# zillow/salve

Measured on AMD Instinct MI355X. Metric: alignment hypotheses/sec (render+verify), higher is better.
Workload: dtype fp16

## Files before the change

### include/salve_hip.h

```cpp
#ifndef SALVE_HIP_H
#define SALVE_HIP_H

#include <stddef.h>
#include <stdint.h>

#ifdef __cplusplus
extern "C" {
#endif

typedef enum {
    SALVE_OK = 0,
    SALVE_ERR_BAD_ARG = -1,
    SALVE_ERR_UNSUPPORTED = -2,
    SALVE_ERR_HIP = -3,
    SALVE_ERR_WORKSPACE = -4
} salve_status_t;

#define SALVE_HIP_ABI_VERSION 7

#define SALVE_STATUS_WALK_FAILED 1
#define SALVE_STATUS_FP16_RANGE 2
#define SALVE_STATUS_BAD_HYPOTHESIS 4

#define SALVE_STATUS_LAYOUT_THICKNESS 8
// ... 78 lines not shown
    int32_t reserved;
    float R[4], t[2];
    double s;
} salve_layout_pose_t;
int salve_layout_pose(const double* room_xy, const int64_t* room_off, int64_t n_room_xy, const double* wdo_xy, const uint8_t* wdo_type,
                      const int64_t* wdo_off, int64_t n_wdo, int32_t n_panos, const salve_layout_pose_t* recs, int32_t n,
                      double bev_tx, double bev_ty, double bev_scale, int32_t line_width, salve_layout_t* layouts, int32_t* poly_xy,
                      int32_t poly_cap, int32_t* segs, int32_t seg_cap, int32_t* status, void* stream);

int salve_bev_export_u8(const uint32_t* bev, int32_t n, int32_t bev_h, int32_t bev_w, uint8_t* out, void* stream);

typedef struct {
    int64_t bev_offset;
    int32_t slot;
    int32_t chan;
} salve_tile_job_t;

#define SALVE_TILE_F32_NCHW 0
#define SALVE_TILE_F16_NHWC 1
#define SALVE_TILE_U8X4 2

int salve_bev_tiles(const uint32_t* bev, int32_t bev_h, int32_t bev_w, const salve_tile_job_t* jobs, int32_t n_jobs,
                    const int32_t* coef_y, const int32_t* coef_x, int32_t resize, int32_t crop, const float* lut,
                    void* out, int32_t out_format, int32_t out_c, void* stream);

typedef struct {
    int32_t crop_y, crop_x;
    int32_t flags;
    int32_t reserved;
} salve_tile_aug_t;
#define SALVE_TILE_HFLIP 1
#define SALVE_TILE_VFLIP 2
int salve_bev_tiles_aug(const uint32_t* bev, int32_t bev_h, int32_t bev_w, const salve_tile_job_t* jobs, const salve_tile_aug_t* aug,
                        int32_t n_jobs, const int32_t* coef_y, const int32_t* coef_x, int32_t resize, int32_t crop, const float* lut,
                        float* out, int32_t out_c, void* stream);

#define SALVE_TILE_F32_NHWC 3
#define SALVE_TILE_BF16_NHWC 4
int salve_bev_train_tiles(const uint32_t* bev_a, int32_t n_bev_a, const uint32_t* bev_b, int32_t n_bev_b, int32_t bev_h, int32_t bev_w,
                          const salve_tile_job_t* jobs_a, const salve_tile_job_t* jobs_b, int32_t per_sample, const salve_tile_aug_t* aug,
                          int32_t batch, const int32_t* coef_y, const int32_t* coef_x, int32_t resize, int32_t crop, const float* lut,
                          void* out, int32_t out_format, int32_t out_c, int32_t* status, void* stream);

int salve_bev_tile_pairs(const uint32_t* bev_a, const uint32_t* bev_b, int32_t bev_h, int32_t bev_w, const salve_tile_job_t* jobs_a,
                         const salve_tile_job_t* jobs_b, int32_t n_pairs, const int32_t* coef_y, const int32_t* coef_x, int32_t resize,
                         int32_t crop, const float* lut, void* out, int32_t out_c, int32_t b_pretiled, void* stream);

int salve_bev_densify_tiles(const salve_bev_config_t* cfg, int32_t n, uint32_t* out_bev, const salve_tile_job_t* jobs_a, const salve_tile_job_t* jobs_b,
                            const uint32_t* tiles_b, const int32_t* coef_y, const int32_t* coef_x, int32_t resize, int32_t crop, const float* lut,
                            void* out, int32_t out_c, int32_t* status, void* workspace, size_t workspace_bytes, void* stream);

#define SALVE_OP_CONV 0
#define SALVE_OP_MAXPOOL 1
#define SALVE_OP_AVGPOOL_FC 2
#define SALVE_NET_INPUT (-1)
#define SALVE_NO_BUF (-2)

typedef struct {
    int32_t op;
    int32_t in_buf, out_buf, res_buf;
    int32_t Hi, Wi, Cin;
    int32_t Ho, Wo, Cout;
    int32_t KH, KW, stride, pad;
    int32_t relu, reserved;
    int64_t w_off;
    int64_t b_off;
    int64_t ktab_off;
    int32_t in2_buf, Cin2, stride2, Hi2, Wi2, reserved2;
} salve_resnet_op_t;

#define SALVE_RESNET_CONV_IGEMM_ONLY 1
#define SALVE_RESNET_CONV8_WHEREVER 2
#define SALVE_RESNET_ROUND_ROBIN_TILES 4
#define SALVE_RESNET_NO_STEM_FUSE 8
#define SALVE_RESNET_NO_BLOCK_FUSE 16
#define SALVE_RESNET_NO_PROJ_FUSE 32
#define SALVE_RESNET_NO_CHAIN 64
#define SALVE_RESNET_CHAIN_EXPAND_ONLY 128
#define SALVE_RESNET_CHAIN_16_WAVES 256
#define SALVE_RESNET_CHAIN_NO_SPLIT 512
#define SALVE_RESNET_CHAIN_STORE_ALL 1024
#define SALVE_RESNET_NO_TRANSPOSED_TILES 2048
#define SALVE_RESNET_NO_NEXT_FUSE 4096
#define SALVE_RESNET_ALL_FLAGS 8191

void* salve_resnet_create(int32_t num_layers, int32_t in_channels, const salve_resnet_op_t* ops, int32_t n_ops,
                          const void* weights_f16, size_t weights_bytes, const float* params_f32, size_t params_bytes,
                          const int32_t* ktab, size_t ktab_entries, int32_t flags);
void salve_resnet_destroy(void* handle);
int salve_resnet_num_layers(void* handle);
size_t salve_resnet_workspace_bytes(void* handle, int32_t batch);
int salve_resnet_forward(void* handle, const void* input, int32_t batch, float* logits, void* workspace,
                         size_t workspace_bytes, int32_t* status, void* stream);

void* salve_resnet_f32_create(int32_t num_layers, int32_t in_channels, const salve_resnet_op_t* ops, int32_t n_ops,
                              const float* weights_f32, size_t weights_bytes, const float* params_f32, size_t params_bytes,
                              const int32_t* ktab, size_t ktab_entries, int32_t flags);
void salve_resnet_f32_destroy(void* handle);
size_t salve_resnet_f32_workspace_bytes(void* handle, int32_t batch);
int salve_resnet_f32_forward(void* handle, const float* input, int32_t batch, float* logits, void* workspace,
                             size_t workspace_bytes, int32_t* status, void* stream);

typedef struct {
    int32_t batch, Hi, Wi, Cin, Ho, Wo, Cout, KH, KW, stride, pad;
} salve_conv_desc_t;
#define SALVE_CONV_FWD 0
#define SALVE_CONV_DGRAD 1
#define SALVE_CONV_WGRAD 2
size_t salve_conv_f32_workspace_bytes(const salve_conv_desc_t* d, int32_t pass);
int salve_conv_f32_forward(const salve_conv_desc_t* d, const float* x, const float* w, float* y, void* ws, size_t ws_bytes, void* stream);
int salve_conv_f32_backward_data(const salve_conv_desc_t* d, const float* dy, const float* w, float* dx, void* ws, size_t ws_bytes,
                                 void* stream);
int salve_conv_f32_backward_weight(const salve_conv_desc_t* d, const float* x, const float* dy, float* dw, void* ws, size_t ws_bytes,
                                   void* stream);

size_t salve_conv_bf16_workspace_bytes(const salve_conv_desc_t* d, int32_t pass);
int salve_conv_bf16_forward(const salve_conv_desc_t* d, const uint16_t* x, const uint16_t* w, uint16_t* y, void* ws, size_t ws_bytes,
                            void* stream);
int salve_conv_bf16_backward_data(const salve_conv_desc_t* d, const uint16_t* dy, const uint16_t* w, uint16_t* dx, void* ws, size_t ws_bytes,
                                  void* stream);
int salve_conv_bf16_backward_weight(const salve_conv_desc_t* d, const uint16_t* x, const uint16_t* dy, float* dw, void* ws, size_t ws_bytes,
                                    void* stream);

typedef struct {
    int32_t rows, C, flags;
    float eps, momentum;
} salve_bn_desc_t;
#define SALVE_BN_RELU 1
#define SALVE_BN_ADD 2
#define SALVE_BN_EVAL 4
#define SALVE_BN_FWD 0
#define SALVE_BN_BWD 1
size_t salve_bn_workspace_bytes(const salve_bn_desc_t* d, int32_t pass);
int salve_bn_f32_forward(const salve_bn_desc_t* d, const float* x, const float* residual, const float* gamma, const float* beta,
                         float* running_mean, float* running_var, float* y, float* save_mean, float* save_invstd, void* ws, size_t ws_bytes,
                         void* stream);
int salve_bn_f32_backward(const salve_bn_desc_t* d, const float* dy, const float* x, const float* y, const float* gamma, const float* save_mean,
                          const float* save_invstd, float* dx, float* dres, float* dgamma, float* dbeta, void* ws, size_t ws_bytes, void* stream);
int salve_bn_bf16_forward(const salve_bn_desc_t* d, const uint16_t* x, const uint16_t* residual, const float* gamma, const float* beta,
                          float* running_mean, float* running_var, uint16_t* y, float* save_mean, float* save_invstd, void* ws, size_t ws_bytes,
                          void* stream);
int salve_bn_bf16_backward(const salve_bn_desc_t* d, const uint16_t* dy, const uint16_t* x, const uint16_t* y, const float* gamma,
                           const float* save_mean, const float* save_invstd, uint16_t* dx, uint16_t* dres, float* dgamma, float* dbeta, void* ws,
                           size_t ws_bytes, void* stream);

#define SALVE_ADAM_CHUNK 4096
typedef struct {
    float* param;
    const float* grad;
    float* exp_avg;
    float* exp_avg_sq;
    uint16_t* shadow_bf16;
    int64_t n;
    float step_size, sqrt_bc2, beta1, beta2, eps, weight_decay, one_minus_beta1, one_minus_beta2;
} salve_adam_segment_t;
typedef struct {
    int32_t segment, reserved;
    int64_t offset;
} salve_adam_chunk_t;
int salve_adam_step(const salve_adam_segment_t* table, int32_t n_segments, const salve_adam_chunk_t* chunk_map, int32_t n_chunks,
                    const salve_adam_segment_t* host_table, const salve_adam_chunk_t* host_chunk_map, void* stream);

#define SALVE_HEAD_MAX_CLASSES 16
typedef struct {
    int32_t B, HW, C, K, flags;
} salve_head_desc_t;
typedef struct {
// ... 24 lines not shown
```

### salve_amd/_lib.py

```python

from __future__ import annotations

import ctypes
from pathlib import Path

import numpy as np

import os

LIB_PATH = Path(os.environ.get("SALVE_HIP_LIB") or (Path(__file__).resolve().parent / "libsalve_hip.so"))

SALVE_OK = 0
EXPECTED_ABI = 7
TILE_F32_NCHW = 0
TILE_F16_NHWC = 1
TILE_U8X4 = 2
TILE_F32_NHWC = 3
TILE_BF16_NHWC = 4

EXPORTED_SYMBOLS = (
    "salve_hip_version",
    "salve_last_error",
    "salve_bev_workspace_bytes",
    "salve_bev_pano_index_bytes",
    "salve_bev_pano_index_build",
    "salve_bev_render_batch",
    "salve_bev_scatter",
    "salve_bev_densify",
    "salve_bev_scatter_points",
    "salve_zorder_winners",
    "salve_remove_hallucinated",
    "salve_bev_keys_from_pixels",
    "salve_bev_export_u8",
    "salve_layout_rasterise",
    "salve_bev_tiles",
    "salve_bev_tile_pairs",
    "salve_bev_densify_tiles",
    "salve_resize_rgb_u8",
    "salve_resnet_create",
    "salve_resnet_destroy",
    "salve_resnet_workspace_bytes",
    "salve_resnet_forward",
    "salve_resnet_num_layers",
    "salve_resnet_f32_create",
    "salve_resnet_f32_destroy",
    "salve_resnet_f32_workspace_bytes",
    "salve_resnet_f32_forward",
    "salve_bev_tiles_aug",
    "salve_conv_f32_workspace_bytes",
    "salve_conv_f32_forward",
    "salve_conv_f32_backward_data",
    "salve_conv_f32_backward_weight",
    "salve_conv_bf16_workspace_bytes",
    "salve_conv_bf16_forward",
    "salve_conv_bf16_backward_data",
    "salve_conv_bf16_backward_weight",
    "salve_bn_workspace_bytes",
    "salve_bn_f32_forward",
    "salve_bn_f32_backward",
    "salve_bn_bf16_forward",
    "salve_bn_bf16_backward",
    "salve_bev_train_tiles",
    "salve_bev_pano_index_update",
    "salve_layout_pose",
    "salve_adam_step",
    "salve_head_workspace_bytes",
    "salve_head_f32_forward",
    "salve_head_f32_backward",
    "salve_head_bf16_forward",
    "salve_head_bf16_backward",
)
RESNET_CONV_IGEMM_ONLY, RESNET_CONV8_WHEREVER, RESNET_ROUND_ROBIN_TILES, RESNET_NO_STEM_FUSE, RESNET_NO_BLOCK_FUSE = 1, 2, 4, 8, 16
RESNET_NO_PROJ_FUSE, RESNET_NO_CHAIN, RESNET_CHAIN_EXPAND_ONLY, RESNET_CHAIN_16_WAVES, RESNET_CHAIN_NO_SPLIT = 32, 64, 128, 256, 512
RESNET_CHAIN_STORE_ALL, RESNET_NO_TRANSPOSED_TILES, RESNET_NO_NEXT_FUSE = 1024, 2048, 4096
STATUS_WALK_FAILED = 1
STATUS_FP16_RANGE = 2
STATUS_BAD_HYPOTHESIS = 4
STATUS_LAYOUT_THICKNESS = 8
STATUS_BAD_TILE_JOB = 16
STATUS_BAD_PANO_SLOT = 32
STATUS_BAD_LAYOUT = 64


class BevConfig(ctypes.Structure):

    _fields_ = [
        ("pano_h", ctypes.c_int32), ("pano_w", ctypes.c_int32), ("crop_rows", ctypes.c_int32),
        ("bev_h", ctypes.c_int32), ("bev_w", ctypes.c_int32), ("mask_k", ctypes.c_int32),
        ("depth_scale", ctypes.c_float), ("out_flags", ctypes.c_int32),
        ("win_xmin", ctypes.c_double), ("win_xmax", ctypes.c_double),
        ("win_ymin", ctypes.c_double), ("win_ymax", ctypes.c_double),
        ("img_tx", ctypes.c_double), ("img_ty", ctypes.c_double), ("img_scale", ctypes.c_double),
        ("rot_pre", ctypes.c_double * 4),
        ("z_lo", ctypes.c_double * 2), ("z_hi", ctypes.c_double * 2),
        ("z_min", ctypes.c_double), ("n_slices", ctypes.c_int32), ("reserved1", ctypes.c_int32),
    ]


HYP_DTYPE = np.dtype(
    [("pano_idx", "<i4"), ("surface", "<i4"), ("R", "<f4", (4,)), ("t", "<f4", (2,)), ("apply_pose", "<i4"),
     ("reserved", "<i4")]
)
TILE_JOB_DTYPE = np.dtype([("bev_offset", "<i8"), ("slot", "<i4"), ("chan", "<i4")])
LAYOUT_DTYPE = np.dtype([("n_poly", "<i4"), ("poly_off", "<i4"), ("n_seg", "<i4"), ("seg_off", "<i4")])
LAYOUT_POSE_DTYPE = np.dtype([("pano", "<i4"), ("poly_off", "<i4"), ("seg_off", "<i4"), ("reserved", "<i4"), ("R", "<f4", (4,)), ("t", "<f4", (2,)),
                              ("s", "<f8")])
TILE_AUG_DTYPE = np.dtype([("crop_y", "<i4"), ("crop_x", "<i4"), ("flags", "<i4"), ("reserved", "<i4")])
TILE_HFLIP, TILE_VFLIP = 1, 2
assert LAYOUT_POSE_DTYPE.itemsize == 48 and HYP_DTYPE.itemsize == 40 and TILE_JOB_DTYPE.itemsize == 16 and TILE_AUG_DTYPE.itemsize == 16

CONV_FWD, CONV_DGRAD, CONV_WGRAD = 0, 1, 2
SALVE_ERR_BAD_ARG, SALVE_ERR_UNSUPPORTED = -1, -2


class ConvDesc(ctypes.Structure):

    _fields_ = [(n, ctypes.c_int32) for n in ("batch", "Hi", "Wi", "Cin", "Ho", "Wo", "Cout", "KH", "KW", "stride", "pad")]


BN_RELU, BN_ADD, BN_EVAL = 1, 2, 4
BN_FWD, BN_BWD = 0, 1


class BnDesc(ctypes.Structure):

    _fields_ = [("rows", ctypes.c_int32), ("C", ctypes.c_int32), ("flags", ctypes.c_int32), ("eps", ctypes.c_float),
                ("momentum", ctypes.c_float)]


ADAM_CHUNK = 4096
ADAM_SEGMENT_DTYPE = np.dtype([("param", "<u8"), ("grad", "<u8"), ("exp_avg", "<u8"), ("exp_avg_sq", "<u8"), ("shadow_bf16", "<u8"), ("n", "<i8"),
                               ("step_size", "<f4"), ("sqrt_bc2", "<f4"), ("beta1", "<f4"), ("beta2", "<f4"), ("eps", "<f4"),
                               ("weight_decay", "<f4"), ("one_minus_beta1", "<f4"), ("one_minus_beta2", "<f4")])
ADAM_CHUNK_DTYPE = np.dtype([("segment", "<i4"), ("reserved", "<i4"), ("offset", "<i8")])
assert ADAM_SEGMENT_DTYPE.itemsize == 80 and ADAM_CHUNK_DTYPE.itemsize == 16

HEAD_MAX_CLASSES = 16
HEAD_ACCUMULATE_LOSS = 1
HEAD_FWD, HEAD_BWD = 0, 1
HEAD_METER_DTYPE = np.dtype([("total", "<i8", (HEAD_MAX_CLASSES,)), ("correct", "<i8", (HEAD_MAX_CLASSES,)), ("loss_sum", "<f8"), ("loss_rows", "<i8"),
                             ("bad_targets", "<i8")])
assert HEAD_METER_DTYPE.itemsize == 280


class HeadDesc(ctypes.Structure):

    _fields_ = [(n, ctypes.c_int32) for n in ("B", "HW", "C", "K", "flags")]


_lib = None


class SalveHipError(RuntimeError):
    pass


def load() -> ctypes.CDLL:
# ... 132 lines not shown
```

### salve_amd/csrc/conv8.h

```cpp

constexpr int C8_THREADS = 512;
constexpr int C8_BM = 256, C8_BN = 256, C8_KS = 64;
constexpr int C8_HALF_E = 128 * C8_KS;

#define C8_MFMA(B_, A_, C_) { C_ = __builtin_amdgcn_mfma_f32_16x16x32_f16(B_, A_, C_, 0, 0, 0); }

template <bool POINTWISE, bool SRC2>
__global__ __launch_bounds__(C8_THREADS, 2) void conv8_kernel(ConvArgs p) {
    constexpr int BM = C8_BM, BN = C8_BN, KS = C8_KS;
    constexpr int LDC = BN + 8;
    constexpr int RING_E = 8 * C8_HALF_E, C_E = BM * LDC;
    __shared__ __attribute__((aligned(1024))) uint16_t smem[RING_E > C_E ? RING_E : C_E];

    int m_tile, n_tile;
    if (!xcd_tile(blockIdx.x, p.m_tiles, p.n_tiles, p.xcd_contig, m_tile, n_tile)) return;
    const int tid = threadIdx.x, lane = tid & 63, wave = __builtin_amdgcn_readfirstlane(tid >> 6);
    const int wr = wave >> 2, wc = wave & 3;
    const int m0 = m_tile * BM, n0 = n_tile * BN;
    const int r8 = tid >> 3;
    const int chunk = (tid & 7) ^ ((r8 >> 1) & 7);

    int iy0[2][2], ix0[2][2];
    const uint16_t* rowp[2][2];
    const uint16_t* rowp2[2][2];
// ... 123 lines not shown
    asm volatile("s_waitcnt vmcnt(8)" ::: "memory");
    __builtin_amdgcn_s_barrier();
    if (wave >= 4) __builtin_amdgcn_s_barrier();
    for (int kt = 0; kt < nkt; kt++) {
        C8_PHASE_HEAD({ C8_READ_A(kt, 0); C8_READ_B(bf0, kt, 1); }, C8_STAGE(kt + 1, 2));
        C8_WAIT_BARRIER();
        C8_MULT(0, bf0, 0);
        __builtin_amdgcn_s_barrier();
        C8_PHASE_HEAD({ C8_READ_B(bf1, kt, 2); }, C8_STAGE(kt + 1, 3));
        C8_WAIT_BARRIER();
        C8_MULT(0, bf1, 1);
        __builtin_amdgcn_s_barrier();
        C8_PHASE_HEAD({ C8_READ_A(kt, 3); }, C8_STAGE(kt + 2, 0));
        C8_WAIT_BARRIER();
        C8_MULT(1, bf1, 1);
        __builtin_amdgcn_s_barrier();
        C8_STAGE(kt + 2, 1);
        C8_WAIT_BARRIER();
        C8_MULT(1, bf0, 0);
        __builtin_amdgcn_s_barrier();
    }
    if (wave < 4) __builtin_amdgcn_s_barrier();
#undef C8_STAGE
#undef C8_READ_A
#undef C8_READ_B
#undef C8_MULT
#undef C8_WAIT_BARRIER
#undef C8_PHASE_HEAD
#undef C8_SLOT
    asm volatile("s_waitcnt vmcnt(0)" ::: "memory");
    __builtin_amdgcn_s_barrier();

    uint16_t* Cs = smem;
    constexpr int CH_PER_ROW = BN / 8;
    constexpr int C_ITERS = (BM * CH_PER_ROW) / C8_THREADS;
    float4 bias_v[4];
#pragma unroll
    for (int j = 0; j < 4; j++) bias_v[j] = *reinterpret_cast<const float4*>(p.bias + n0 + wc * 64 + j * 16 + 4 * frag_q);
    constexpr int ROW_STEP = C8_THREADS / CH_PER_ROW;
    const int crow = tid / CH_PER_ROW, cch = tid % CH_PER_ROW;
    const long long coff = (long long)(m0 + crow) * p.Cout + n0 + cch * 8;
    const int cstep = ROW_STEP * p.Cout;
    if (p.res) {
        constexpr int RB = 8;
#pragma unroll
        for (int it0 = 0; it0 < C_ITERS; it0 += RB) {
            uint4 rv[RB];
#pragma unroll
            for (int u = 0; u < RB; u++) {
                const bool in = m0 + crow + (it0 + u) * ROW_STEP < p.M;
                rv[u] = *reinterpret_cast<const uint4*>(p.res + (in ? coff + (long long)(it0 + u) * cstep : (long long)m0 * p.Cout + n0));
            }
#pragma unroll
            for (int u = 0; u < RB; u++)
                *reinterpret_cast<uint4*>(Cs + (crow + (it0 + u) * ROW_STEP) * LDC + cch * 8) = rv[u];
        }
        __syncthreads();
    }
    float amax = 0.f;
    float amin = 0.f;
    const float lo = p.relu ? 0.f : -65504.f;
#pragma unroll
    for (int j = 0; j < 4; j++) {
        const int ncol = wc * 64 + j * 16 + 4 * frag_q;
        const float4 bias = bias_v[j];
#pragma unroll
        for (int i = 0; i < 8; i++) {
            const int mrow = wr * 128 + i * 16 + frag_row;
            uint2* cell = reinterpret_cast<uint2*>(Cs + mrow * LDC + ncol);
            f32x4 v = acc[i][j] + vec4(bias);
            if (p.res) v += vec4(*cell);
            *cell = pack4_lo(amax, amin, v, lo);
        }
    }
    if (!p.relu) amax = fmaxf(amax, -amin);
    report_range(p.status, amax);
    __syncthreads();
#pragma unroll 4
    for (int it = 0; it < C_ITERS; it++) {
        if (m0 + crow + it * ROW_STEP < p.M)
            *reinterpret_cast<uint4*>(p.out + coff + (long long)it * cstep) = *reinterpret_cast<const uint4*>(Cs + (crow + it * ROW_STEP) * LDC + cch * 8);
    }
}
```

### salve_amd/csrc/resnet.hip

```cpp
#include <hip/hip_runtime.h>
#include <stdint.h>
#include <stdlib.h>
#include <string.h>
#include <type_traits>
#include <vector>

#include "../../include/salve_hip.h"
#include "salve_common.h"

namespace {

typedef __attribute__((__ext_vector_type__(8))) _Float16 act8;
typedef __attribute__((__ext_vector_type__(4))) float f32x4;

constexpr int BM = 128;
constexpr int BK = 64;
constexpr int CONV_THREADS = 256;

struct ConvArgs {
    const uint16_t* in;
    const uint16_t* w;
    const float* bias;
    const uint16_t* res;
    uint16_t* out;
// ... 741 lines not shown
#pragma unroll
            for (int it = 0; it < C_ITERS; it++) {
                const int id = tl + it * BN_THREADS;
                const int m = id / CH_PER_ROW, ch = id % CH_PER_ROW;
                const int oy = img_y(m >> 4, m & 15), ox = img_x(m >> 4, m & 15);
                bool keep = ox < p.W && oy < p.H;
                if constexpr (NEXT) keep = keep && (!p.y_even || (((oy | ox) & 1) == 0));
                if (keep)
                    store16_stream(yimg + ((long long)oy * p.W + ox) * C4 + nc * 128 + ch * 8, *reinterpret_cast<const uint4*>(Cs + m * LDC + ch * 8));
            }
            if constexpr (NEXT) {
                if (nc == 0) {
#pragma unroll
                    for (int i = 0; i < RT; i++)
#pragma unroll
                        for (int j = 0; j < MIDN / 32; j++) acc4[i][j] = f32x4{0.f, 0.f, 0.f, 0.f};
                }
                GEMM4_KTILE(0, BsC);
                if (nc == C4 / 128 - 1) {
                    GEMM4_KTILE(64, T2);
                } else {
                    asm volatile("s_waitcnt lgkmcnt(0)" ::: "memory");
                    asm volatile("s_barrier" ::: "memory");
                    ISSUE_WD(2 * nc + 1, BsC);
                    asm volatile("s_waitcnt vmcnt(0)" ::: "memory");
                    asm volatile("s_barrier" ::: "memory");
                    GEMM4_KTILE(64, BsC);
                }
                asm volatile("s_waitcnt lgkmcnt(0)" ::: "memory");
            }
            __syncthreads();
        }
        if constexpr (NEXT) {
#pragma unroll
            for (int j = 0; j < MIDN / 32; j++) {
                const int ncol = (wc * (MIDN / 32) + j) * 16 + 4 * frag_q;
                const float4 bias = *reinterpret_cast<const float4*>(p.bd + ncol);
#pragma unroll
                for (int i = 0; i < RT; i++) {
                    const int m = (wr * RT + i) * 16 + frag_row;
                    *reinterpret_cast<uint2*>(Cs + m * LDC + ncol) = pack4<true>(amax, acc4[i][j] + vec4(bias));
                }
            }
            __syncthreads();
            uint16_t* timg = p.t1n + (long long)b * p.H * p.W * MIDN;
            constexpr int CPR = MIDN / 8;
            int tl = tid;
            asm volatile("" : "+v"(tl));
#pragma unroll
            for (int it = 0; it < (MO * CPR) / BN_THREADS; it++) {
                const int id = tl + it * BN_THREADS;
                const int m = id / CPR, ch = id % CPR;
                const int oy = img_y(m >> 4, m & 15), ox = img_x(m >> 4, m & 15);
                if (ox < p.W && oy < p.H)
                    store16_stream(timg + ((long long)oy * p.W + ox) * MIDN + ch * 8, *reinterpret_cast<const uint4*>(Cs + m * LDC + ch * 8));
            }
        }
#undef ISSUE_WD
#undef GEMM4_KTILE
    }
    report_range(p.status, amax);
}

struct ResnetHandle {
    std::vector<salve_resnet_op_t> ops;
    uint16_t* d_weights = nullptr;
    float* d_params = nullptr;
    int32_t* d_ktab = nullptr;
    uint16_t* d_zeros = nullptr;
    size_t max_act_elems = 0;
    int n_bufs = 0;
    int num_layers = 0, in_channels = 0, ncls = 0;
    std::vector<int> fused;
    std::vector<int> wide;
    bool wide_auto = false;
    std::vector<int> stem;
    int xcd_contig = 1;
    std::vector<int> chain;
    int n_cus = 256;
    int chain_split = 1;
    int chain_dbg = 0, chain_waves = 8;
    std::vector<int> y_even;
    std::vector<int> next;
    int no_transposed_tiles = 0;
};

static bool chain_shape(int mid, int midn) { return (mid == 128 && (midn == 128 || midn == 256)) || (mid == 256 && midn == 256); }
static bool expand_shape(int mid) { return mid == 128 || mid == 256; }

enum { WIDE_OFF = 0, WIDE_256_K64_S2 = 4, WIDE_128_K64_S1 = 5, WIDE_PC_128 = 6, WIDE_8PHASE = 7, WIDE_AUTO = 8 };

static bool is_pow2(int v) { return v > 0 && (v & (v - 1)) == 0; }

static int choose_wide(const salve_resnet_op_t& o, int force) {
    if (o.op != SALVE_OP_CONV || force == WIDE_OFF) return WIDE_OFF;
    const bool pointwise = o.KH == 1 && o.KW == 1 && o.stride == 1 && o.pad == 0;
    const int K = o.KH * o.KW * o.Cin + (o.in2_buf != SALVE_NO_BUF ? o.Cin2 : 0);
    if (!pointwise && (!is_pow2(o.Cin) || o.Cin < 64)) return WIDE_OFF;
    if (K < 128 || K % 64 != 0) return WIDE_OFF;
    if (force == WIDE_8PHASE || force == WIDE_AUTO) {
        const bool fits = o.Cout % 256 == 0 && is_pow2(o.Cin) && o.Cin >= 64 && (o.in2_buf == SALVE_NO_BUF || o.Cin2 % 64 == 0);
        return (fits && (force == WIDE_8PHASE || K >= 512)) ? WIDE_8PHASE : WIDE_OFF;
    }
    if (force == WIDE_256_K64_S2) return o.Cout % 256 == 0 ? force : WIDE_OFF;
    return o.Cout % 128 == 0 ? force : WIDE_OFF;
}

bool check_op(const salve_resnet_op_t& o) {
    if (o.op == SALVE_OP_CONV) {
        if (o.Cout % 64 != 0) return salve_fail("conv: Cout must be a multiple of 64");
        if (o.Cin % 8 != 0) return salve_fail("conv: Cin must be a multiple of 8");
        if ((o.KH * o.KW * o.Cin) % BK != 0) return salve_fail("conv: KH*KW*Cin must be a multiple of 64");
        if (o.in2_buf != SALVE_NO_BUF) {
            if (o.KH != 1 || o.KW != 1 || o.stride != 1 || o.pad != 0 || o.res_buf != SALVE_NO_BUF)
                return salve_fail("conv: a second source needs a 1x1 / stride 1 / pad 0 convolution without residual");
            if (o.Cin2 <= 0 || o.Cin2 % BK != 0 || o.stride2 < 1 || (o.Hi2 - 1) / o.stride2 + 1 != o.Ho || (o.Wi2 - 1) / o.stride2 + 1 != o.Wo)
                return salve_fail("conv: bad second-source geometry");
        }
    } else if (o.op == SALVE_OP_MAXPOOL) {
        if (o.Cin % 8 != 0) return salve_fail("maxpool: C must be a multiple of 8");
    } else if (o.op == SALVE_OP_AVGPOOL_FC) {
        if (o.Cout < 1 || o.Cout > 8) return salve_fail("fc: 1..8 classes supported");
        if (o.Cin % 8 != 0) return salve_fail("fc: C must be a multiple of 8");
    } else {
        return salve_fail("unknown op");
    }
    return true;
}

}

extern "C" {



void* salve_resnet_create(int32_t num_layers, int32_t in_channels, const salve_resnet_op_t* ops, int32_t n_ops,
                          const void* weights_f16, size_t weights_bytes, const float* params_f32, size_t params_bytes,
                          const int32_t* ktab, size_t ktab_entries, int32_t flags) {
    if (!ops || n_ops <= 0 || !weights_f16 || !params_f32 || !ktab) {
        salve_fail("salve_resnet_create: null argument");
        return nullptr;
    }
    if (flags & ~SALVE_RESNET_ALL_FLAGS) {
        salve_fail("salve_resnet_create: unknown bit in flags (SALVE_RESNET_*): a caller written for another ABI version");
        return nullptr;
    }
    ResnetHandle* h = new ResnetHandle();
    h->num_layers = num_layers;
    h->in_channels = in_channels;
    for (int i = 0; i < n_ops; i++) {
        if (!check_op(ops[i])) { delete h; return nullptr; }
        h->ops.push_back(ops[i]);
        const salve_resnet_op_t& o = ops[i];
        if (o.op != SALVE_OP_AVGPOOL_FC) {
            const size_t e = (size_t)o.Ho * o.Wo * o.Cout;
            if (e > h->max_act_elems) h->max_act_elems = e;
            if (o.out_buf + 1 > h->n_bufs) h->n_bufs = o.out_buf + 1;
        } else {
            h->ncls = o.Cout;
        }
    }
    h->wide.assign(h->ops.size(), 0);
    {
        int mode = (flags & SALVE_RESNET_CONV_IGEMM_ONLY) ? WIDE_OFF : ((flags & SALVE_RESNET_CONV8_WHEREVER) ? WIDE_8PHASE : WIDE_AUTO);
#ifdef SALVE_BUILD_ABLATIONS
        if (const char* e = getenv("SALVE_CONV_WIDE")) mode = e[0] == 'd' ? WIDE_256_K64_S2 : (e[0] == 'e' ? WIDE_128_K64_S1 : (e[0] == 'f' ? WIDE_PC_128 : mode));
#endif
        h->wide_auto = mode == WIDE_AUTO;
        for (size_t i = 0; i < h->ops.size(); i++) h->wide[i] = choose_wide(h->ops[i], mode);
    }
    h->xcd_contig = (flags & SALVE_RESNET_ROUND_ROBIN_TILES) ? 0 : 1;
    h->no_transposed_tiles = (flags & SALVE_RESNET_NO_TRANSPOSED_TILES) ? 1 : 0;
    h->stem.assign(h->ops.size(), 0);
    {
        const bool enable = !(flags & SALVE_RESNET_NO_STEM_FUSE);
        for (size_t i = 0; enable && i + 1 < h->ops.size(); i++) {
            const salve_resnet_op_t &a = h->ops[i], &b = h->ops[i + 1];
            if (a.op != SALVE_OP_CONV || b.op != SALVE_OP_MAXPOOL) continue;
            bool k_order = a.Cin == 8;
            if ((a.Cin == 16 || a.Cin == 24) && a.KH == 7 && a.KW == 8 && (size_t)a.ktab_off + (size_t)(a.Cin / 8) * 7 * 8 <= ktab_entries) {
                k_order = true;
                for (int q = 0; q < (a.Cin / 8) * 7 * 8 && k_order; q++) {
                    const int g = q / 56, kh = (q % 56) / 8, kw = q % 8;
                    k_order = ktab[a.ktab_off + q] == ((kh & 0xFF) | ((kw & 0xFF) << 8) | ((8 * g) << 16));
                }
            }
            const bool shape = a.KH == 7 && a.KW == 8 && a.stride == 2 && a.pad == 3 && (a.Cin == 8 || a.Cin == 16 || a.Cin == 24) && k_order && a.Cout == 64 && a.relu &&
                               a.res_buf == SALVE_NO_BUF && a.in2_buf == SALVE_NO_BUF && b.in_buf == a.out_buf && b.Cin == 64 &&
                               a.Hi % 4 == 0 && a.Wi % 4 == 0 && a.Wi == STEM_W && (a.Hi / 4) % STEM_R == 0 &&
                               a.Ho == a.Hi / 2 && a.Wo == a.Wi / 2 && b.Ho == a.Hi / 4 && b.Wo == a.Wi / 4;
            bool dead = shape;
            for (size_t k = i + 2; dead && k < h->ops.size(); k++) {
                const salve_resnet_op_t& o = h->ops[k];
                if (o.in_buf == a.out_buf || (o.op == SALVE_OP_CONV && (o.res_buf == a.out_buf || o.in2_buf == a.out_buf))) dead = false;
                if (o.out_buf == a.out_buf) break;
            }
            if (dead) h->stem[i] = 1;
        }
    }
    h->fused.assign(h->ops.size(), 0);
    {
        const bool enable = !(flags & SALVE_RESNET_NO_BLOCK_FUSE);
        for (size_t i = 0; enable && i + 2 < h->ops.size(); i++) {
            const salve_resnet_op_t &a = h->ops[i], &b = h->ops[i + 1], &c = h->ops[i + 2];
            if (a.op != SALVE_OP_CONV || b.op != SALVE_OP_CONV || c.op != SALVE_OP_CONV) continue;
            const int mid = a.Cout;
            const bool shapes = a.KH == 1 && a.KW == 1 && a.stride == 1 && a.pad == 0 && a.relu && a.res_buf == SALVE_NO_BUF && a.Cin == 4 * mid &&
                                b.KH == 3 && b.KW == 3 && b.stride == 1 && b.pad == 1 && b.relu && b.res_buf == SALVE_NO_BUF && b.Cin == mid && b.Cout == mid &&
                                b.in_buf == a.out_buf && a.in2_buf == SALVE_NO_BUF && c.in2_buf == SALVE_NO_BUF && c.KH == 1 && c.KW == 1 && c.stride == 1 && c.pad == 0 && c.relu && c.Cin == mid &&
                                c.Cout == 4 * mid && c.in_buf == b.out_buf && c.res_buf == a.in_buf && c.out_buf != a.in_buf && a.in_buf >= 0 &&
                                a.Hi == c.Ho && a.Wi == c.Wo && b.Hi == a.Hi && b.Ho == a.Hi;
            const bool proj = a.KH == 1 && a.KW == 1 && a.stride == 1 && a.pad == 0 && a.relu && a.res_buf == SALVE_NO_BUF && a.in2_buf == SALVE_NO_BUF &&
                              a.Cin == mid && b.KH == 3 && b.KW == 3 && b.stride == 1 && b.pad == 1 && b.relu && b.res_buf == SALVE_NO_BUF &&
                              b.in2_buf == SALVE_NO_BUF && b.Cin == mid && b.Cout == mid && b.in_buf == a.out_buf && c.KH == 1 && c.KW == 1 && c.stride == 1 &&
                              c.pad == 0 && c.relu && c.res_buf == SALVE_NO_BUF && c.Cin == mid && c.Cout == 4 * mid && c.in_buf == b.out_buf &&
                              c.in2_buf == a.in_buf && c.Cin2 == mid && c.stride2 == 1 && c.out_buf != a.in_buf && a.in_buf >= 0 && a.Hi == c.Ho &&
                              a.Wi == c.Wo && b.Hi == a.Hi && b.Ho == a.Hi && c.Hi2 == a.Hi && c.Wi2 == a.Wi && !(flags & SALVE_RESNET_NO_PROJ_FUSE);
            if (!(shapes || proj) || mid != 64 || a.Hi % 8 != 0) continue;
            bool dead = true;
            for (int which = 0; which < 2 && dead; which++) {
                const int id = which ? b.out_buf : a.out_buf;
                for (size_t k = i + 3; k < h->ops.size(); k++) {
                    const salve_resnet_op_t& o = h->ops[k];
                    if (o.in_buf == id || (o.op == SALVE_OP_CONV && (o.res_buf == id || o.in2_buf == id))) { dead = false; break; }
                    if (o.out_buf == id) break;
                }
            }
            if (dead) { h->fused[i] = shapes ? 1 : 2; i += 2; }
        }
    }
    h->next.assign(h->ops.size(), 0);
    for (size_t i = 0; !(flags & SALVE_RESNET_NO_NEXT_FUSE) && i + 3 < h->ops.size(); i++) {
        if (h->fused[i] != 1) continue;
        const salve_resnet_op_t &a = h->ops[i], &c = h->ops[i + 2], &n = h->ops[i + 3];
        const int mid = a.Cout;
        const bool fits = n.op == SALVE_OP_CONV && n.KH == 1 && n.KW == 1 && n.stride == 1 && n.pad == 0 && n.relu && n.res_buf == SALVE_NO_BUF &&
                          n.in2_buf == SALVE_NO_BUF && n.in_buf == c.out_buf && n.Cin == 4 * mid && n.Cout == 2 * mid && n.Hi == c.Ho && n.Wi == c.Wo &&
                          n.out_buf >= 0 && n.out_buf != c.out_buf && n.out_buf != a.in_buf && !h->fused[i + 3];
        if (!fits) continue;
        bool even = !(flags & SALVE_RESNET_CHAIN_STORE_ALL) && c.Ho == c.Wo && !(c.Ho & 1), any = false;
        for (size_t k = i + 4; even && k < h->ops.size(); k++) {
            const salve_resnet_op_t& o = h->ops[k];
            if (o.in_buf == c.out_buf || (o.op == SALVE_OP_CONV && o.res_buf == c.out_buf)) even = false;
            if (o.op == SALVE_OP_CONV && o.in2_buf == c.out_buf) {
                if (o.stride2 == 2 && o.Hi2 == c.Ho && o.Wi2 == c.Wo) any = true; else even = false;
            }
            if (o.op != SALVE_OP_AVGPOOL_FC && o.out_buf == c.out_buf) break;
        }
        h->next[i] = (even && any) ? 2 : 1;
    }
    h->chain.assign(h->ops.size(), 0);
    {
        const int mode = (flags & SALVE_RESNET_NO_CHAIN) ? 0 : ((flags & SALVE_RESNET_CHAIN_EXPAND_ONLY) ? 1 : 2);
        for (size_t i = 0; mode > 0 && i < h->ops.size(); i++) {
            const salve_resnet_op_t& c = h->ops[i];
// ... 136 lines not shown
            else hipLaunchKernelGGL((bottleneck_kernel<128, 4>), dim3((unsigned)grid), dim3(BN_THREADS), 0, s, a);
            SALVE_HIP_CHECK(hipGetLastError());
            oi += with_next ? 3 : 2;
            continue;
        }
        if (o.op == SALVE_OP_CONV && h->chain[oi]) {
            const bool chained = h->chain[oi] == 2;
            const salve_resnet_op_t& on = h->ops[chained ? oi + 1 : oi];
            ChainArgs a;
            a.t2 = buf(o.in_buf); a.x = buf(o.res_buf); a.y = buf(o.out_buf);
            a.wc = h->d_weights + o.w_off; a.bc = h->d_params + o.b_off;
            a.t1n = chained ? buf(on.out_buf) : nullptr;
            a.wa = chained ? h->d_weights + on.w_off : nullptr;
            a.ba = chained ? h->d_params + on.b_off : nullptr;
            a.zeros = h->d_zeros;
            const long long M = (long long)batch * o.Ho * o.Wo;
            if (M > 0x7FFFFFFFll) { salve_fail("batch too large"); return SALVE_ERR_BAD_ARG; }
            a.M = (int)M;
            a.status = status;
            a.y_even_w = h->y_even[oi] ? o.Wo : 0;
            a.dbg = h->chain_dbg;
            const int mid = o.Cin, midn = chained ? on.Cout : 0;
            const bool wide = h->chain_waves == 16 && mid == 128 && (!chained || midn == 128);
            const bool split = !wide && h->chain_split && (mid == 256 || (chained && midn == 256));
            const int rows = wide ? 256 : 128;
            a.n_tiles = (int)((M + rows - 1) / rows);
            const unsigned grid = (unsigned)(a.n_tiles < h->n_cus ? a.n_tiles : h->n_cus);
            const dim3 blk((wide || split) ? 1024 : 512);
            if (split && chained && mid == 128) hipLaunchKernelGGL((expand_chain_kernel<128, 256, 8, true, 2, 16, 2>), dim3(grid), blk, 0, s, a);
            else if (split && chained) hipLaunchKernelGGL((expand_chain_kernel<256, 256, 5, true, 2, 16, 2>), dim3(grid), blk, 0, s, a);
            else if (split) hipLaunchKernelGGL((expand_chain_kernel<256, 256, 12, false, 2, 16, 2>), dim3(grid), blk, 0, s, a);
            else if (wide && chained) hipLaunchKernelGGL((expand_chain_kernel<128, 128, 6, true, 2, 16>), dim3(grid), blk, 0, s, a);
            else if (wide) hipLaunchKernelGGL((expand_chain_kernel<128, 128, 7, false, 2, 16>), dim3(grid), blk, 0, s, a);
            else if (chained && mid == 128 && midn == 128) hipLaunchKernelGGL((expand_chain_kernel<128, 128, 12, true>), dim3(grid), blk, 0, s, a);
            else if (chained && mid == 128 && midn == 256) hipLaunchKernelGGL((expand_chain_kernel<128, 256, 8, true>), dim3(grid), blk, 0, s, a);
            else if (chained && mid == 256 && midn == 256) hipLaunchKernelGGL((expand_chain_kernel<256, 256, 5, true>), dim3(grid), blk, 0, s, a);
            else if (!chained && mid == 128) hipLaunchKernelGGL((expand_chain_kernel<128, 128, 14, false>), dim3(grid), blk, 0, s, a);
            else if (!chained && mid == 256) hipLaunchKernelGGL((expand_chain_kernel<256, 256, 12, false>), dim3(grid), blk, 0, s, a);
            else { salve_fail("expand_chain: unsupported shape"); return SALVE_ERR_UNSUPPORTED; }
            SALVE_HIP_CHECK(hipGetLastError());
            if (chained) oi += 1;
            continue;
        }
        if (o.op == SALVE_OP_CONV) {
            ConvArgs a;
            a.in = buf(o.in_buf);
            a.w = h->d_weights + o.w_off;
            a.bias = h->d_params + o.b_off;
            a.res = o.res_buf != SALVE_NO_BUF ? buf(o.res_buf) : nullptr;
            a.out = buf(o.out_buf);
            a.ktab = h->d_ktab + o.ktab_off;
            a.zeros = h->d_zeros;
            a.status = status;
            a.xcd_contig = h->xcd_contig;
            a.B = batch; a.Hi = o.Hi; a.Wi = o.Wi; a.Cin = o.Cin; a.Ho = o.Ho; a.Wo = o.Wo; a.Cout = o.Cout;
            a.stride = o.stride; a.pad = o.pad; a.K = o.KH * o.KW * o.Cin; a.relu = o.relu;
            const bool src2 = o.in2_buf != SALVE_NO_BUF;
            a.in2 = src2 ? buf(o.in2_buf) : nullptr;
            a.Hi2 = o.Hi2; a.Wi2 = o.Wi2; a.Cin2 = o.Cin2; a.stride2 = o.stride2;
            a.nkt1 = a.K / BK;
            if (src2) a.K += o.Cin2;
            const long long M = (long long)batch * o.Ho * o.Wo;
            if (M > 0x7FFFFFFFll) { salve_fail("batch too large"); return SALVE_ERR_BAD_ARG; }
            a.M = (int)M;
            a.KW = o.KW;
            a.cin_log2 = 0;
            while ((1 << a.cin_log2) < o.Cin) a.cin_log2++;
            const bool few_tiles = h->wide[oi] == WIDE_8PHASE && h->wide_auto && ((M + 255) / 256) * (long long)(o.Cout / 256) < 1536;
            if (h->wide[oi] != WIDE_OFF && !few_tiles) {
                const int cfg = h->wide[oi];
                const int bn = (cfg == WIDE_256_K64_S2 || cfg == WIDE_8PHASE) ? 256 : 128;
                a.m_tiles = (int)((M + C8_BM - 1) / C8_BM);
                a.n_tiles = o.Cout / bn;
                const unsigned grid = (unsigned)(((a.m_tiles + 7) / 8) * 8 * a.n_tiles);
                const bool pw = o.KH == 1 && o.KW == 1 && o.stride == 1 && o.pad == 0;
#ifdef SALVE_BUILD_ABLATIONS
#define WIDE_LAUNCH(BN_, KS_, NS_)                                                                                                  \
    {                                                                                                                               \
        if (src2) hipLaunchKernelGGL((conv_wide_kernel<BN_, KS_, NS_, true, true>), dim3(grid), dim3(WIDE_THREADS), 0, s, a);       \
        else if (pw) hipLaunchKernelGGL((conv_wide_kernel<BN_, KS_, NS_, true, false>), dim3(grid), dim3(WIDE_THREADS), 0, s, a);   \
        else hipLaunchKernelGGL((conv_wide_kernel<BN_, KS_, NS_, false, false>), dim3(grid), dim3(WIDE_THREADS), 0, s, a);          \
    }
#endif
                if (cfg == WIDE_8PHASE) {
                    if (src2) hipLaunchKernelGGL((conv8_kernel<true, true>), dim3(grid), dim3(C8_THREADS), 0, s, a);
                    else if (pw) hipLaunchKernelGGL((conv8_kernel<true, false>), dim3(grid), dim3(C8_THREADS), 0, s, a);
                    else hipLaunchKernelGGL((conv8_kernel<false, false>), dim3(grid), dim3(C8_THREADS), 0, s, a);
                }
#ifdef SALVE_BUILD_ABLATIONS
                else if (cfg == WIDE_PC_128) {
                    if (src2) hipLaunchKernelGGL((conv_pc_kernel<true, true>), dim3(grid), dim3(PC_THREADS), 0, s, a);
                    else if (pw) hipLaunchKernelGGL((conv_pc_kernel<true, false>), dim3(grid), dim3(PC_THREADS), 0, s, a);
                    else hipLaunchKernelGGL((conv_pc_kernel<false, false>), dim3(grid), dim3(PC_THREADS), 0, s, a);
                } else if (cfg == WIDE_256_K64_S2) WIDE_LAUNCH(256, 64, 2)
                else WIDE_LAUNCH(128, 64, 1)
#undef WIDE_LAUNCH
#endif
                SALVE_HIP_CHECK(hipGetLastError());
                continue;
            }
            a.m_tiles = (int)((M + BM - 1) / BM);
            const int bn = (o.Cout % 128 == 0) ? 128 : 64;
            a.n_tiles = o.Cout / bn;
            const unsigned grid = (unsigned)(((a.m_tiles + 7) / 8) * 8 * a.n_tiles);
            const bool pointwise = o.KH == 1 && o.KW == 1 && o.stride == 1 && o.pad == 0;
            if (src2 && bn == 128) {
                hipLaunchKernelGGL((conv_igemm_kernel<128, true, true>), dim3(grid), dim3(CONV_THREADS), 0, s, a);
            } else if (src2) {
                hipLaunchKernelGGL((conv_igemm_kernel<64, true, true>), dim3(grid), dim3(CONV_THREADS), 0, s, a);
            } else if (bn == 128 && pointwise) {
                hipLaunchKernelGGL((conv_igemm_kernel<128, true>), dim3(grid), dim3(CONV_THREADS), 0, s, a);
            } else if (bn == 128) {
                hipLaunchKernelGGL((conv_igemm_kernel<128, false>), dim3(grid), dim3(CONV_THREADS), 0, s, a);
            } else if (pointwise) {
                hipLaunchKernelGGL((conv_igemm_kernel<64, true>), dim3(grid), dim3(CONV_THREADS), 0, s, a);
            } else {
                hipLaunchKernelGGL((conv_igemm_kernel<64, false>), dim3(grid), dim3(CONV_THREADS), 0, s, a);
            }
        } else if (o.op == SALVE_OP_MAXPOOL) {
            const long long total = (long long)batch * o.Ho * o.Wo * (o.Cin / 8);
            hipLaunchKernelGGL(maxpool_kernel, dim3((unsigned)((total + 255) / 256)), dim3(256), 0, s, buf(o.in_buf), buf(o.out_buf),
                               batch, o.Hi, o.Wi, o.Cin, o.Ho, o.Wo);
        } else {
            hipLaunchKernelGGL(avgpool_fc_kernel, dim3(batch), dim3(256), 0, s, buf(o.in_buf), o.Hi * o.Wi,
                               o.Cin, h->d_params + o.w_off, h->d_params + o.b_off, o.Cout, logits);
        }
        SALVE_HIP_CHECK(hipGetLastError());
    }
    return SALVE_OK;
}

}
```

Before: 60480.

## Add persistent conv8 kernel that prefetches next tile during epilogue

Adds a persistent variant of the 256x256 8-phase conv GEMM kernel, launched with one block per CU (rounded to a multiple of 8). Each block loops over tiles, and near the end of each K loop it sets up addressing for the next tile and begins staging its first K slices, overlapping the next tile's loads with the current tile's epilogue. The epilogue now writes through a small 32-row LDS slab in eight steps and prefetches residuals in two batches, which shrinks the LDS footprint. The change removes per-tile launch and prologue cost but limits parallelism to one block per CU, even though launch bounds allow two, and it adds barrier-heavy epilogue logic. A flag disables the new path.

New measurement: 60450 (median of 2 runs). Within noise of the previous version (-0.1%).

```diff
diff --git a/include/salve_hip.h b/include/salve_hip.h
--- a/include/salve_hip.h
+++ b/include/salve_hip.h
@@ -184,7 +184,8 @@
 #define SALVE_RESNET_CHAIN_STORE_ALL 1024
 #define SALVE_RESNET_NO_TRANSPOSED_TILES 2048
 #define SALVE_RESNET_NO_NEXT_FUSE 4096
-#define SALVE_RESNET_ALL_FLAGS 8191
+#define SALVE_RESNET_NO_CONV8_PERSIST 16384
+#define SALVE_RESNET_ALL_FLAGS (8191 | 16384)
 
 void* salve_resnet_create(int32_t num_layers, int32_t in_channels, const salve_resnet_op_t* ops, int32_t n_ops,
                           const void* weights_f16, size_t weights_bytes, const float* params_f32, size_t params_bytes,
diff --git a/salve_amd/_lib.py b/salve_amd/_lib.py
--- a/salve_amd/_lib.py
+++ b/salve_amd/_lib.py
@@ -73,6 +73,7 @@
 RESNET_CONV_IGEMM_ONLY, RESNET_CONV8_WHEREVER, RESNET_ROUND_ROBIN_TILES, RESNET_NO_STEM_FUSE, RESNET_NO_BLOCK_FUSE = 1, 2, 4, 8, 16
 RESNET_NO_PROJ_FUSE, RESNET_NO_CHAIN, RESNET_CHAIN_EXPAND_ONLY, RESNET_CHAIN_16_WAVES, RESNET_CHAIN_NO_SPLIT = 32, 64, 128, 256, 512
 RESNET_CHAIN_STORE_ALL, RESNET_NO_TRANSPOSED_TILES, RESNET_NO_NEXT_FUSE = 1024, 2048, 4096
+RESNET_NO_CONV8_PERSIST = 16384
 STATUS_WALK_FAILED = 1
 STATUS_FP16_RANGE = 2
 STATUS_BAD_HYPOTHESIS = 4
diff --git a/salve_amd/csrc/conv8.h b/salve_amd/csrc/conv8.h
--- a/salve_amd/csrc/conv8.h
+++ b/salve_amd/csrc/conv8.h
@@ -229,3 +229,279 @@
             *reinterpret_cast<uint4*>(p.out + coff + (long long)it * cstep) = *reinterpret_cast<const uint4*>(Cs + (crow + it * ROW_STEP) * LDC + cch * 8);
     }
 }
+
+__device__ __forceinline__ void lds_write16(uint16_t* p, uint4 v) {
+    act8 t = __builtin_bit_cast(act8, v);
+    asm volatile("" : "+v"(t));
+    *reinterpret_cast<act8*>(p) = t;
+}
+
+template <bool POINTWISE, bool SRC2, bool RES>
+__global__ __launch_bounds__(C8_THREADS, 2) void conv8p_kernel(ConvArgs p) {
+    constexpr int BM = C8_BM, BN = C8_BN, KS = C8_KS;
+    constexpr int LDC = BN + 8, SLAB = 32;
+    constexpr int RING_E = 8 * C8_HALF_E;
+    __shared__ __attribute__((aligned(1024))) uint16_t smem[RING_E + SLAB * LDC];
+    uint16_t* const Cs = smem + RING_E;
+
+    const int tid = threadIdx.x, lane = tid & 63, wave = __builtin_amdgcn_readfirstlane(tid >> 6);
+    const int wr = wave >> 2, wc = wave & 3;
+    const int r8 = tid >> 3;
+    const int chunk = (tid & 7) ^ ((r8 >> 1) & 7);
+    const int nkt = p.K / KS;
+    const int n_ids = ((p.m_tiles + 7) >> 3) * 8 * p.n_tiles;
+    const int id_step = gridDim.x;
+
+    int id = blockIdx.x, m_tile = 0, n_tile = 0;
+    while (id < n_ids && !xcd_tile(id, p.m_tiles, p.n_tiles, p.xcd_contig, m_tile, n_tile)) id += id_step;
+    if (id >= n_ids) return;
+
+    int iy0[2][2], ix0[2][2];
+    const uint16_t* rowp[2][2];
+    const uint16_t* rowp2[2][2];
+    const uint16_t* wrow[2][2];
+    bool st_live = true;
+    int st_off = 0;
+#define C8P_SETUP(MT, NT)                                                                                              \
+    {                                                                                                                  \
+        int r8o_ = r8;                                                                                                 \
+        asm volatile("" : "+v"(r8o_));                                                                                 \
+        const int ch8_ = ((tid & 7) ^ ((r8o_ >> 1) & 7)) * 8;                                                          \
+        const int sm0_ = (MT) * BM, sn0_ = (NT) * BN;                                                                  \
+        _Pragma("unroll") for (int s = 0; s < 2; s++)                                                                  \
+            _Pragma("unroll") for (int i = 0; i < 2; i++) {                                                            \
+                const int m = sm0_ + i * 128 + s * 64 + r8o_;                                                          \
+                const bool valid = m < p.M;                                                                            \
+                rowp[s][i] = nullptr;                                                                                  \
+                rowp2[s][i] = nullptr;                                                                                 \
+                iy0[s][i] = ix0[s][i] = 0;                                                                             \
+                if (SRC2 && valid) {                                                                                   \
+                    const int ox = m % p.Wo, t = m / p.Wo, oy = t % p.Ho, b = t / p.Ho;                                \
+                    rowp2[s][i] = p.in2 + (((long long)b * p.Hi2 + (long long)oy * p.stride2) * p.Wi2 + (long long)ox * p.stride2) * p.Cin2 + ch8_; \
+                }                                                                                                      \
+                if (POINTWISE) {                                                                                       \
+                    rowp[s][i] = valid ? p.in + (long long)m * p.Cin + ch8_ : nullptr;                                 \
+                } else {                                                                                               \
+                    const int mm = valid ? m : 0;                                                                      \
+                    const int ox = mm % p.Wo, t = mm / p.Wo, oy = t % p.Ho, b = t / p.Ho;                              \
+                    iy0[s][i] = valid ? oy * p.stride - p.pad : -100000;                                               \
+                    ix0[s][i] = ox * p.stride - p.pad;                                                                 \
+                    rowp[s][i] = p.in + (((long long)b * p.Hi + (valid ? iy0[s][i] : 0)) * p.Wi + ix0[s][i]) * p.Cin + ch8_; \
+                }                                                                                                      \
+                wrow[s][i] = p.w + (long long)(sn0_ + ((r8o_ + 64 * i) >> 5) * 64 + s * 32 + (r8o_ & 31)) * p.K + ch8_; \
+            }                                                                                                          \
+    }
+#define C8P_SLOT(G, KIND) (smem + ((((G) & 1) << 2) + (KIND)) * C8_HALF_E)
+#define C8P_STAGE(G, KTL, KIND)                                                                                        \
+    do {                                                                                                               \
+        uint16_t* dst_ = C8P_SLOT(G, KIND) + wave * 8 * KS;                                                            \
+        const int kt_ = (KTL);                                                                                         \
+        const bool live_ = st_live;                                                                                    \
+        constexpr int s_ = ((KIND) == 2 || (KIND) == 3) ? 1 : 0;                                                       \
+        if ((KIND) == 0 || (KIND) == 3) {                                                                              \
+            int dy_ = 0, dx_ = 0, delta_ = 0;                                                                          \
+            if (!POINTWISE) {                                                                                          \
+                const int k0_ = kt_ * KS;                                                                              \
+                const int tap_ = k0_ >> p.cin_log2;                                                                    \
+                dy_ = tap_ / p.KW;                                                                                     \
+                dx_ = tap_ - dy_ * p.KW;                                                                               \
+                delta_ = (dy_ * p.Wi + dx_) * p.Cin + (k0_ & (p.Cin - 1));                                             \
+            }                                                                                                          \
+            _Pragma("unroll") for (int i = 0; i < 2; i++) {                                                            \
+                const uint16_t* src = p.zeros;                                                                         \
+                if (live_) {                                                                                           \
+                    if (SRC2 && kt_ >= p.nkt1) {                                                                       \
+                        if (rowp2[s_][i]) src = rowp2[s_][i] + (kt_ - p.nkt1) * KS;                                    \
+                    } else if (POINTWISE) {                                                                            \
+                        if (rowp[s_][i]) src = rowp[s_][i] + kt_ * KS;                                                 \
+                    } else if ((unsigned)(iy0[s_][i] + dy_) < (unsigned)p.Hi && (unsigned)(ix0[s_][i] + dx_) < (unsigned)p.Wi) { \
+                        src = rowp[s_][i] + delta_;                                                                    \
+                    }                                                                                                  \
+                }                                                                                                      \
+                __builtin_amdgcn_global_load_lds((global_cptr)src, (lds_ptr)(dst_ + i * 64 * KS), 16, 0, 0);           \
+            }                                                                                                          \
+        } else {                                                                                                       \
+            _Pragma("unroll") for (int i = 0; i < 2; i++) {                                                            \
+                const uint16_t* src = live_ ? wrow[s_][i] + kt_ * KS : p.zeros;                                        \
+                __builtin_amdgcn_global_load_lds((global_cptr)src, (lds_ptr)(dst_ + i * 64 * KS), 16, 0, 0);           \
+            }                                                                                                          \
+        }                                                                                                              \
+    } while (0)
+
+    const int frag_row = lane & 15, frag_q = lane >> 4;
+    const int frag_sw = (frag_row >> 1) & 7;
+    const int a_off = (wr * 64 + frag_row) * KS, b_off = (wc * 32 + frag_row) * KS;
+    const int pos0 = ((0 * 4 + frag_q) ^ frag_sw) * 8, pos1 = ((1 * 4 + frag_q) ^ frag_sw) * 8;
+    act8 af[4][2], bf0[2][2], bf1[2][2];
+#define C8P_READ_A(G, KIND)                                                                                            \
+    {                                                                                                                  \
+        const uint16_t* h_ = C8P_SLOT(G, KIND) + a_off;                                                                \
+        _Pragma("unroll") for (int i = 0; i < 4; i++) {                                                                \
+            af[i][0] = *reinterpret_cast<const act8*>(h_ + i * 16 * KS + pos0);                                        \
+            af[i][1] = *reinterpret_cast<const act8*>(h_ + i * 16 * KS + pos1);                                        \
+        }                                                                                                              \
+    }
+#define C8P_READ_B(DST, G, KIND)                                                                                       \
+    {                                                                                                                  \
+        const uint16_t* h_ = C8P_SLOT(G, KIND) + b_off;                                                                \
+        _Pragma("unroll") for (int j = 0; j < 2; j++) {                                                                \
+            DST[j][0] = *reinterpret_cast<const act8*>(h_ + j * 16 * KS + pos0);                                       \
+            DST[j][1] = *reinterpret_cast<const act8*>(h_ + j * 16 * KS + pos1);                                       \
+        }                                                                                                              \
+    }
+#define C8P_MULT(QA, BF, QB)                                                                                           \
+    {                                                                                                                  \
+        asm volatile("s_waitcnt lgkmcnt(0)" ::: "memory");                                                             \
+        C8_PRIO(1);                                                                                                    \
+        _Pragma("unroll") for (int ks = 0; ks < 2; ks++)                                                               \
+            _Pragma("unroll") for (int i = 0; i < 4; i++)                                                              \
+                _Pragma("unroll") for (int j = 0; j < 2; j++) C8_MFMA(BF[j][ks], af[i][ks], acc[(QA) * 4 + i][(QB) * 2 + j]) \
+        C8_PRIO(0);                                                                                                    \
+    }
+#define C8P_WAIT_BARRIER()                                                                                             \
+    {                                                                                                                  \
+        if (kt) C8_VMWAIT();                                                                                           \
+        __builtin_amdgcn_s_barrier();                                                                                  \
+    }
+#define C8P_LDS_BARRIER()                                                                                              \
+    {                                                                                                                  \
+        asm volatile("s_waitcnt lgkmcnt(0)" ::: "memory");                                                             \
+        __builtin_amdgcn_s_barrier();                                                                                  \
+    }
+
+    C8P_SETUP(m_tile, n_tile);
+    C8P_STAGE(0, 0, 0);
+    C8P_STAGE(0, 0, 1);
+    C8P_STAGE(0, 0, 2);
+    C8P_STAGE(0, 0, 3);
+    C8P_STAGE(1, 1, 0);
+    C8P_STAGE(1, 1, 1);
+    asm volatile("s_waitcnt vmcnt(0)" ::: "memory");
+    __builtin_amdgcn_s_barrier();
+
+    int gpar = 0;
+    for (;;) {
+        const int m0 = m_tile * BM, n0 = n_tile * BN;
+        int nid = id + id_step, nm_tile = 0, nn_tile = 0;
+        while (nid < n_ids && !xcd_tile(nid, p.m_tiles, p.n_tiles, p.xcd_contig, nm_tile, nn_tile)) nid += id_step;
+        const bool has_next = nid < n_ids;
+
+        f32x4 acc[8][4];
+#pragma unroll
+        for (int i = 0; i < 8; i++)
+#pragma unroll
+            for (int j = 0; j < 4; j++) acc[i][j] = f32x4{0.f, 0.f, 0.f, 0.f};
+
+        if (wave >= 4) __builtin_amdgcn_s_barrier();
+        for (int kt = 0; kt < nkt; kt++) {
+            const int g = gpar + kt;
+            { C8P_READ_A(g, 0); C8P_READ_B(bf0, g, 1); }
+            C8P_STAGE(g + 1, kt + 1 - st_off, 2);
+            C8P_WAIT_BARRIER();
+            C8P_MULT(0, bf0, 0);
+            __builtin_amdgcn_s_barrier();
+            { C8P_READ_B(bf1, g, 2); }
+            C8P_STAGE(g + 1, kt + 1 - st_off, 3);
+            C8P_WAIT_BARRIER();
+            C8P_MULT(0, bf1, 1);
+            __builtin_amdgcn_s_barrier();
+            if (kt == nkt - 2) {
+                st_live = has_next;
+                st_off = nkt;
+                if (has_next) C8P_SETUP(nm_tile, nn_tile);
+            }
+            { C8P_READ_A(g, 3); }
+            C8P_STAGE(g + 2, kt + 2 - st_off, 0);
+            C8P_WAIT_BARRIER();
+            C8P_MULT(1, bf1, 1);
+            __builtin_amdgcn_s_barrier();
+            C8P_STAGE(g + 2, kt + 2 - st_off, 1);
+            C8P_WAIT_BARRIER();
+            C8P_MULT(1, bf0, 0);
+            __builtin_amdgcn_s_barrier();
+        }
+        if (wave < 4) __builtin_amdgcn_s_barrier();
+        st_off = 0;
+
+        int tido = tid;
+        asm volatile("" : "+v"(tido));
+        const int crow = tido >> 5, cch = tido & 31;
+        const int efrag_row = tido & 15, efrag_q = (tido >> 4) & 3;
+        const uint16_t* const res_t = p.res + ((long long)m0 * p.Cout + n0);
+        uint16_t* const out_t = p.out + ((long long)m0 * p.Cout + n0);
+        const unsigned coff = (unsigned)(crow * p.Cout + cch * 8);
+        float4 bias_v[4];
+#pragma unroll
+        for (int j = 0; j < 4; j++) bias_v[j] = *reinterpret_cast<const float4*>(p.bias + n0 + wc * 64 + j * 16 + 4 * efrag_q);
+        uint4 rv[8][2];
+#define C8P_RES_LOAD(S0)                                                                                               \
+    if (RES) {                                                                                                       \
+        _Pragma("unroll") for (int s = (S0); s < (S0) + 4; s++)                                                        \
+            _Pragma("unroll") for (int it = 0; it < 2; it++) {                                                         \
+                const int row = it * 128 + s * 16;                                                                     \
+                const bool in = m0 + crow + row < p.M;    \
+                rv[s][it] = *reinterpret_cast<const uint4*>(res_t + (in ? coff + (unsigned)(row * p.Cout) : 0u));      \
+            }                                                                                                          \
+    }
+#define C8P_SLAB_OUT(S)                                                                                                \
+    _Pragma("unroll") for (int it = 0; it < 2; it++) {                                                                 \
+        const int row = it * 128 + (S) * 16;                                                                           \
+        const uint4 v = lds_read16(Cs + (crow + it * 16) * LDC + cch * 8);                                             \
+        if (m0 + crow + row < p.M) *reinterpret_cast<uint4*>(out_t + (coff + (unsigned)(row * p.Cout))) = v;           \
+    }
+#define C8P_RES_LANDED(S0)                                                                                             \
+    if (RES) {                                                                                                         \
+        _Pragma("unroll") for (int s = (S0); s < (S0) + 4; s++)                                                        \
+            _Pragma("unroll") for (int it = 0; it < 2; it++)                                                           \
+                asm volatile("" : "+v"(rv[s][it].x), "+v"(rv[s][it].y), "+v"(rv[s][it].z), "+v"(rv[s][it].w));         \
+    }
+        C8P_RES_LOAD(0)
+        asm volatile("s_waitcnt vmcnt(0)" ::: "memory");
+        C8P_RES_LANDED(0)
+        float amax = 0.f;
+        float amin = 0.f;
+        const float lo = p.relu ? 0.f : -65504.f;
+#pragma unroll
+        for (int s = 0; s < 8; s++) {
+            if (s > 0) C8P_SLAB_OUT(s - 1)
+            if (s == 2) C8P_RES_LOAD(4)
+            if (s == 4 && RES) {
+                asm volatile("s_waitcnt vmcnt(0)" ::: "memory");
+                C8P_RES_LANDED(4)
+            }
+            if (RES) {
+#pragma unroll
+                for (int it = 0; it < 2; it++) lds_write16(Cs + (crow + it * 16) * LDC + cch * 8, rv[s][it]);
+            }
+            C8P_LDS_BARRIER();
+#pragma unroll
+            for (int j = 0; j < 4; j++) {
+                uint16_t* cell = Cs + (wr * 16 + efrag_row) * LDC + wc * 64 + j * 16 + 4 * efrag_q;
+                f32x4 v = acc[s][j] + vec4(bias_v[j]);
+                if (RES) v += vec4(lds_read8(cell));
+                lds_write8(cell, pack4_lo(amax, amin, v, lo));
+            }
+            C8P_LDS_BARRIER();
+        }
+        C8P_SLAB_OUT(7)
+#undef C8P_SLAB_OUT
+#undef C8P_RES_LOAD
+#undef C8P_RES_LANDED
+        if (!p.relu) amax = fmaxf(amax, -amin);
+        report_range(p.status, amax);
+
+        if (!has_next) break;
+        id = nid;
+        m_tile = nm_tile;
+        n_tile = nn_tile;
+        gpar = (gpar + nkt) & 1;
+    }
+#undef C8P_SETUP
+#undef C8P_SLOT
+#undef C8P_STAGE
+#undef C8P_READ_A
+#undef C8P_READ_B
+#undef C8P_MULT
+#undef C8P_WAIT_BARRIER
+#undef C8P_LDS_BARRIER
+}
diff --git a/salve_amd/csrc/resnet.hip b/salve_amd/csrc/resnet.hip
--- a/salve_amd/csrc/resnet.hip
+++ b/salve_amd/csrc/resnet.hip
@@ -847,6 +847,7 @@
     int chain_dbg = 0, chain_waves = 8;
     std::vector<int> y_even;
     std::vector<int> next;
+    int conv8_persist = 1;
     int no_transposed_tiles = 0;
 };
 
@@ -936,6 +937,7 @@
     }
     h->xcd_contig = (flags & SALVE_RESNET_ROUND_ROBIN_TILES) ? 0 : 1;
     h->no_transposed_tiles = (flags & SALVE_RESNET_NO_TRANSPOSED_TILES) ? 1 : 0;
+    h->conv8_persist = (flags & SALVE_RESNET_NO_CONV8_PERSIST) ? 0 : 1;
     h->stem.assign(h->ops.size(), 0);
     {
         const bool enable = !(flags & SALVE_RESNET_NO_STEM_FUSE);
@@ -1238,7 +1240,15 @@
         else hipLaunchKernelGGL((conv_wide_kernel<BN_, KS_, NS_, false, false>), dim3(grid), dim3(WIDE_THREADS), 0, s, a);          \
     }
 #endif
-                if (cfg == WIDE_8PHASE) {
+                if (cfg == WIDE_8PHASE && h->conv8_persist) {
+                    const unsigned cus8 = (unsigned)(h->n_cus >= 8 ? h->n_cus / 8 * 8 : 8);
+                    const unsigned pgrid = grid < cus8 ? grid : cus8;
+                    if (src2) hipLaunchKernelGGL((conv8p_kernel<true, true, false>), dim3(pgrid), dim3(C8_THREADS), 0, s, a);
+                    else if (pw && a.res) hipLaunchKernelGGL((conv8p_kernel<true, false, true>), dim3(pgrid), dim3(C8_THREADS), 0, s, a);
+                    else if (pw) hipLaunchKernelGGL((conv8p_kernel<true, false, false>), dim3(pgrid), dim3(C8_THREADS), 0, s, a);
+                    else if (a.res) hipLaunchKernelGGL((conv8p_kernel<false, false, true>), dim3(pgrid), dim3(C8_THREADS), 0, s, a);
+                    else hipLaunchKernelGGL((conv8p_kernel<false, false, false>), dim3(pgrid), dim3(C8_THREADS), 0, s, a);
+                } else if (cfg == WIDE_8PHASE) {
                     if (src2) hipLaunchKernelGGL((conv8_kernel<true, true>), dim3(grid), dim3(C8_THREADS), 0, s, a);
                     else if (pw) hipLaunchKernelGGL((conv8_kernel<true, false>), dim3(grid), dim3(C8_THREADS), 0, s, a);
                     else hipLaunchKernelGGL((conv8_kernel<false, false>), dim3(grid), dim3(C8_THREADS), 0, s, a);
```
